# NGWPC/topoflow-glacier

Measured on AMD Instinct MI355X. Metric: cell-updates/sec (nx·ny·steps) on 8192² fp32 grid; % HBM roofline, higher is better.
Workload: dtype f32

## Files before the change

topoflow-glacier_amd/csrc/tfg_fused.hpp:

```cpp
#pragma once

#include <hip/hip_runtime.h>

#include <algorithm>
#include <cmath>
#include <cstddef>
#include <cstdint>

#include "../../include/tfg.h"
#include "tfg_physics.hpp"

namespace tfg_kern {

using tfg::CellDiag;
using tfg::CellOut;
using tfg::CellState;
using tfg::CellStatic;
using tfg::CellStaticF;
using tfg::DevParams;

constexpr int kBlock = 256;
constexpr int kCellsPerThread = 1;
constexpr int kPrefetchFast = 2;
constexpr int kWaves = kBlock / 64;
constexpr int kNumForc = 5;
constexpr int kNumState = 8;
constexpr int kNumHist = 6;
enum { S_HSWE = 0, S_HIWE, S_ECCS, S_ECCI, S_N, S_ALB, S_HSNOW, S_HICE };
enum { F_P = 0, F_T, F_Q, F_PA, F_UZ };
enum { H_HSNOW = 0, H_SM, H_HICE, H_IM, H_MTOT, H_RH };

struct KArgs {
  DevParams p;
  int K;
  int n_catch;
  int64_t n, n_pad;
  const void* io_in;
  double* io_out;
  uint32_t* io_flag;
  uint32_t io_seq;
  int64_t n_step = 0;
  int64_t part_c0 = 0;
};

struct StepAddr {
  int64_t forc, ring, hist, pad_;
};
static_assert(sizeof(StepAddr) == 32, "one aligned scalar load of four dwords reaches forc and ring");

static_assert(offsetof(KArgs, p) == 0, "KArgs::p is read at the start of the kernel-argument segment");
#define TFG_STEP_PARAMS(p)                                                                                  \
  auto p##_ks = (const __attribute__((address_space(4))) DevParams*)__builtin_amdgcn_kernarg_segment_ptr(); \
  asm volatile("" : "+s"(p##_ks));                                                                          \
  const DevParams& p = *(const DevParams*)p##_ks

template <class T, int C> struct alignas(C * sizeof(T)) Pack { T v[C]; };

__device__ __forceinline__ uint32_t lane_off(uint32_t off) {
  asm volatile("" : "+v"(off));
  return off;
}
template <class T, int C>
__device__ __forceinline__ void vload(const T* __restrict__ base, uint32_t i, T (&v)[C]) {
  const uint32_t off = lane_off(i * (uint32_t)sizeof(T));
  const Pack<T, C> x = *reinterpret_cast<const Pack<T, C>*>(reinterpret_cast<const char*>(base) + off);
#pragma unroll
  for (int j = 0; j < C; ++j) v[j] = x.v[j];
}
template <class T, int C>
__device__ __forceinline__ void vstore(T* __restrict__ base, uint32_t i, const T (&v)[C]) {
  const uint32_t off = lane_off(i * (uint32_t)sizeof(T));
  Pack<T, C> x;
#pragma unroll
  for (int j = 0; j < C; ++j) x.v[j] = v[j];
  *reinterpret_cast<Pack<T, C>*>(reinterpret_cast<char*>(base) + off) = x;
}
template <class T>
__device__ __forceinline__ T sload(const T* __restrict__ base, uint32_t off) {
  return *reinterpret_cast<const T*>(reinterpret_cast<const char*>(base) + off);
}
template <class T>
__device__ __forceinline__ void sstore(T* __restrict__ base, uint32_t off, T v) {
  __builtin_nontemporal_store(v, reinterpret_cast<T*>(reinterpret_cast<char*>(base) + off));
}
template <int C> __device__ __forceinline__ void dload(const double* p, uint32_t i, double (&v)[C]) { vload<double, C>(p, i, v); }
template <int C> __device__ __forceinline__ void dstore(double* p, uint32_t i, const double (&v)[C]) { vstore<double, C>(p, i, v); }
template <int C> __device__ __forceinline__ void iload(const int32_t* p, uint32_t i, int32_t (&v)[C]) { vload<int32_t, C>(p, i, v); }
template <int C> __device__ __forceinline__ void istore(int32_t* p, uint32_t i, const int32_t (&v)[C]) { vstore<int32_t, C>(p, i, v); }
template <int C> __device__ __forceinline__ void lload(const int64_t* p, uint32_t i, int64_t (&v)[C]) { vload<int64_t, C>(p, i, v); }
template <int C> __device__ __forceinline__ void lstore(int64_t* p, uint32_t i, const int64_t (&v)[C]) { vstore<int64_t, C>(p, i, v); }

__device__ __forceinline__ void diag_scale(CellDiag& d, const DevParams& p) {
  const double f = p.da_m2 * p.dt, f3600 = p.da_m2 * p.dt * 3600.0;
  d.P *= f;
  d.PR *= f;
  d.PS *= f;
  d.SM *= f3600;
  d.IM *= f3600;
}
__device__ __forceinline__ void diag_zero(CellDiag& d) {
  d.P = d.PR = d.PS = d.SM = d.IM = 0.0;
  d.Pmax = -INFINITY;
}

__device__ __forceinline__ void wave_flush(double* __restrict__ wbins, int cid, const CellDiag& d, bool has) {
  const int lane = threadIdx.x & 63;
  uint64_t pending = __ballot(has);
  while (pending) {
    const int leader = __builtin_ctzll(pending);
    const int c = __shfl(cid, leader);
    const bool mine = has && (cid == c);
    double v0 = mine ? d.P : 0.0, v1 = mine ? d.PR : 0.0, v2 = mine ? d.PS : 0.0;
    double v3 = mine ? d.SM : 0.0, v4 = mine ? d.IM : 0.0, m = mine ? d.Pmax : -INFINITY;
#pragma unroll
    for (int off = 32; off >= 1; off >>= 1) {
      v0 += __shfl_xor(v0, off);
      v1 += __shfl_xor(v1, off);
      v2 += __shfl_xor(v2, off);
      v3 += __shfl_xor(v3, off);
      v4 += __shfl_xor(v4, off);
      m = tfg::npmax(m, __shfl_xor(m, off));
    }
    if (lane == leader) {
      double* b = wbins + 6 * c;
      b[0] += v0; b[1] += v1; b[2] += v2; b[3] += v3; b[4] += v4;
      b[5] = tfg::npmax(b[5], m);
    }
    pending &= ~__ballot(mine);
  }
}

#ifdef TFG_WG_TIMING
static __device__ unsigned long long g_wg_times[TFG_WG_TIMING][3];
#endif
constexpr int kMinWaves = 4;
constexpr int kMinWavesExact = 2;
constexpr int kMinWavesPrec = 4;
template <class R, bool EXACT, bool READ_DEPTHS, bool CATCH, bool QC, int C, bool NS = false, bool PREC = false,
          bool SAT = false>
__global__ __launch_bounds__(kBlock, EXACT ? kMinWavesExact : (PREC ? kMinWavesPrec : kMinWaves)) void k_fused(const KArgs a, const tfg_uniforms* __restrict__ uni,
                                                  const StepAddr* __restrict__ tab,
                                                  const R* __restrict__ forc,
                                                  const R* __restrict__ stat,
                                                  const float* __restrict__ geo,
                                                  const int32_t* __restrict__ catch_id,
                                                  double* __restrict__ st,
                                                  int64_t* __restrict__ tot,
                                                  int32_t* __restrict__ ring,
                                                  R* __restrict__ hist,
                                                  double* __restrict__ slab,
                                                  const R* __restrict__ qcf) {
  extern __shared__ double lds_bins[];
#ifdef TFG_WG_TIMING
  const unsigned long long t_wg0 = wall_clock64();
#endif
  const DevParams& p = a.p;
  const int nb = a.n_catch * 6;
  for (int i = threadIdx.x; i < kWaves * nb; i += kBlock) lds_bins[i] = ((i % 6) == 5) ? -INFINITY : 0.0;
  __syncthreads();
  double* wbins = lds_bins + (threadIdx.x >> 6) * nb;

  const int64_t n_pad = a.n_pad;
  const int64_t ngroups = a.n_step / C;
  const int64_t nchunks = (ngroups + kBlock - 1) / kBlock;
  const int64_t wg = blockIdx.x;
  const int64_t g0 = (wg * nchunks / gridDim.x) * kBlock;
  const int64_t g1 = std::min<int64_t>(((wg + 1) * nchunks / gridDim.x) * kBlock, ngroups);
  const int64_t trips = (g1 - g0 + kBlock - 1) / kBlock;
  const double* geo_d = reinterpret_cast<const double*>(geo + tfg::kGeoF * n_pad) + a.part_c0 / 2;
  float* const alb_f = reinterpret_cast<float*>(st + S_ALB * n_pad) - a.part_c0;

  CellDiag acc;
  diag_zero(acc);

  for (int64_t it = 0; it < trips; ++it) {
    const int64_t g = g0 + it * kBlock + threadIdx.x;
    const bool in = g < g1;
    int32_t cid[C];
    CellDiag cacc[CATCH ? C : 1];
    if constexpr (CATCH) {
#pragma unroll
      for (int j = 0; j < C; ++j) { diag_zero(cacc[j]); cid[j] = 0; }
    }
    if (in) {
      const int64_t c0 = g * C;
      const uint32_t lc = (uint32_t)c0;
      if constexpr (CATCH) iload<C>(catch_id, lc, cid);
      CellStatic SX[EXACT ? C : 1];
      tfg::CellStaticF SF[EXACT ? 1 : C];
      if constexpr (EXACT) {
        const double* gx = reinterpret_cast<const double*>(geo);
        double v[tfg::kStaticPlanes][C];
#pragma unroll
        for (int f = 0; f < tfg::kStaticPlanes; ++f) dload<C>(gx + f * n_pad, lc, v[f]);
#pragma unroll
        for (int j = 0; j < C; ++j) SX[j] = {v[0][j], v[1][j], v[2][j], v[3][j], v[4][j], v[5][j], v[6][j]};
      } else {
        float gv[tfg::kGeoF][C];
#pragma unroll
        for (int f = 0; f < tfg::kGeoF; ++f) vload<float, C>(geo + f * n_pad, lc, gv[f]);
#pragma unroll
        for (int j = 0; j < C; ++j) SF[j] = {gv[0][j], gv[1][j], gv[2][j], gv[3][j], gv[4][j]};
      }
      CellState cs[C];
      {
        double v[C];
        dload<C>(st + S_HSWE * n_pad, lc, v);
#pragma unroll
        for (int j = 0; j < C; ++j) cs[j].h_swe = v[j];
        dload<C>(st + S_HIWE * n_pad, lc, v);
#pragma unroll
        for (int j = 0; j < C; ++j) cs[j].h_iwe = v[j];
        dload<C>(st + S_ECCS * n_pad, lc, v);
#pragma unroll
        for (int j = 0; j < C; ++j) cs[j].Eccs = v[j];
        dload<C>(st + S_ECCI * n_pad, lc, v);
#pragma unroll
        for (int j = 0; j < C; ++j) cs[j].Ecci = v[j];
        dload<C>(st + S_N * n_pad, lc, v);
#pragma unroll
        for (int j = 0; j < C; ++j) cs[j].n = v[j];
        if constexpr (EXACT) {
          dload<C>(st + S_ALB * n_pad, lc, v);
#pragma unroll
          for (int j = 0; j < C; ++j) cs[j].albedo = v[j];
        }
        if constexpr (READ_DEPTHS) {
          dload<C>(st + S_HSNOW * n_pad, lc, v);
#pragma unroll
          for (int j = 0; j < C; ++j) cs[j].h_snow = v[j];
          dload<C>(st + S_HICE * n_pad, lc, v);
#pragma unroll
          for (int j = 0; j < C; ++j) cs[j].h_ice = v[j];
        } else {
#pragma unroll
          for (int j = 0; j < C; ++j) {
            cs[j].h_snow = cs[j].h_swe * p.ws;
            cs[j].h_ice = cs[j].h_iwe * p.wi;
          }
        }
        int64_t t[C];
        lload<C>(tot, lc, t);
#pragma unroll
        for (int j = 0; j < C; ++j) cs[j].tot_q = t[j];
        if constexpr (!EXACT) {
          bool carried = false;
#pragma unroll
          for (int j = 0; j < C; ++j) {
            cs[j].albedo = 0.0;
            carried |= !(cs[j].h_snow > 0.0 || (cs[j].h_snow == 0.0 && (cs[j].h_ice > 0.0 || cs[j].h_ice == 0.0)));
          }
          if (__any(carried)) {
            float fa[C];
            vload<float, C>(alb_f, lc, fa);
#pragma unroll
            for (int j = 0; j < C; ++j) cs[j].albedo = (double)fa[j];
          }
        }
      }
      R qc[C];
      if constexpr (QC) vload<R, C>(qcf, lc, qc);
      else {
#pragma unroll
        for (int j = 0; j < C; ++j) qc[j] = (R)0;
      }
      tfg::DiagF df[EXACT ? 1 : C];
      if constexpr (!EXACT) {
#pragma unroll
        for (int j = 0; j < C; ++j) df[j] = {0.0f, 0.0f, 0.0f, 0.0f, 0.0f, 0.0f};
      }

      struct Frame { R P[C], T[C], Q[C], PA[C], UZ[C]; int32_t q[C]; };
      const char* const fbase = a.io_in ? static_cast<const char*>(a.io_in) : reinterpret_cast<const char*>(forc);
      auto fetch = [&](int k, Frame& f) {
        const StepAddr* ta = tab + (k < a.K ? k : a.K - 1);
        const int64_t fo = ta->forc, ro = ta->ring;
        const R* __restrict__ fr = reinterpret_cast<const R*>(fbase + fo);
        const int32_t* rs = reinterpret_cast<const int32_t*>(reinterpret_cast<const char*>(ring) + ro);
        static_assert(C == 1, "streamed step accesses are per cell");
        static_assert(sizeof(R) == 4 || sizeof(R) == 8, "R is float or double");
        const uint32_t oR = lane_off(lc * (uint32_t)sizeof(R));
        f.P[0] = sload(fr + F_P * n_pad, oR);
        f.T[0] = sload(fr + F_T * n_pad, oR);
        f.Q[0] = sload(fr + F_Q * n_pad, oR);
        f.PA[0] = sload(fr + F_PA * n_pad, oR);
        f.UZ[0] = sload(fr + F_UZ * n_pad, oR);
        f.q[0] = sload(rs, sizeof(R) == 4 ? oR : lane_off(lc * 4u));
      };
      auto advance = [&](int k, const Frame& f) {
        TFG_STEP_PARAMS(p);
        const tfg_uniforms* up = uni + k;
        const tfg_uniforms u = *up;
        int32_t qn[C];
        R o_hs[C], o_sm[C], o_hi[C], o_im[C], o_mt[C], o_rh[C];
#pragma unroll
        for (int j = 0; j < C; ++j) {
          if constexpr (EXACT) {
            CellOut o;
            CellDiag& d = CATCH ? cacc[j] : acc;
            const bool valid = (c0 + j) < a.n;
            const tfg::ParamsAsIs params{p};
            tfg::cell_step_exact<QC>(p, SX[j], u, (double)f.P[j], (double)f.T[j], (double)f.Q[j], (double)f.PA[j],
                                     (double)f.UZ[j], f.q[j], qn[j], cs[j], o, d, valid, (double)qc[j], params);
            o_hs[j] = (R)o.h_snow; o_sm[j] = (R)o.SM; o_hi[j] = (R)o.h_ice;
            o_im[j] = (R)o.IM; o_mt[j] = (R)o.M_total; o_rh[j] = (R)o.RH;
          } else {
            tfg::CellOutF o;
            tfg::cell_step_fast<QC, NS, PREC, SAT>(p, SF[j], up, u, geo_d, n_pad, c0 + j, (float)f.P[j], (float)f.T[j],
                                                   (float)f.Q[j], (float)f.PA[j], (float)f.UZ[j], f.q[j], qn[j], cs[j],
                                                   o, df[j], (float)qc[j]);
            o_hs[j] = (R)o.h_snow; o_sm[j] = (R)o.SM; o_hi[j] = (R)o.h_ice;
            o_im[j] = (R)o.IM; o_mt[j] = (R)o.M_total; o_rh[j] = (R)o.RH;
          }
        }
        const uint32_t oR = lane_off(lc * (uint32_t)sizeof(R));
        const int64_t ro = tab[k].ring, ho = tab[k].hist;
        sstore(reinterpret_cast<int32_t*>(reinterpret_cast<char*>(ring) + ro), sizeof(R) == 4 ? oR : lane_off(lc * 4u), qn[0]);
        R* __restrict__ h = reinterpret_cast<R*>(reinterpret_cast<char*>(hist) + ho);
        sstore(h + H_HSNOW * n_pad, oR, o_hs[0]);
        sstore(h + H_SM * n_pad, oR, o_sm[0]);
        sstore(h + H_HICE * n_pad, oR, o_hi[0]);
        sstore(h + H_IM * n_pad, oR, o_im[0]);
        sstore(h + H_MTOT * n_pad, oR, o_mt[0]);
        sstore(h + H_RH * n_pad, oR, o_rh[0]);
      };
      constexpr int kAhead = (QC || NS || PREC) ? 1 : kPrefetchFast;
      Frame fa, fb;
      fetch(0, fa);
      if constexpr (EXACT) {
        for (int k = 0; k < a.K; ++k) {
          fetch(k + 1, fb);
          advance(k, fa);
          fa = fb;
        }
      } else if constexpr (kAhead == 2) {
        Frame fc;
        fetch(1, fb);
        for (int k = 0; k < a.K; k += 3) {
          fetch(k + 2, fc);
          advance(k, fa);
          fetch(k + 3, fa);
          if (k + 1 < a.K) advance(k + 1, fb);
          fetch(k + 4, fb);
          if (k + 2 < a.K) advance(k + 2, fc);
        }
      } else {
        for (int k = 0; k < a.K; k += 2) {
          fetch(k + 1, fb);
          advance(k, fa);
          fetch(k + 2, fa);
          if (k + 1 < a.K) advance(k + 1, fb);
        }
      }
      if (a.io_in) {
        const int fidx = uni[0].frame, hidx = uni[0].hist;
        R* __restrict__ fr = const_cast<R*>(forc) + (int64_t)fidx * kNumForc * n_pad;
        const uint32_t oR = lane_off(lc * (uint32_t)sizeof(R));
        sstore(fr + F_P * n_pad, oR, fa.P[0]);
        sstore(fr + F_T * n_pad, oR, fa.T[0]);
        sstore(fr + F_Q * n_pad, oR, fa.Q[0]);
        sstore(fr + F_PA * n_pad, oR, fa.PA[0]);
        sstore(fr + F_UZ * n_pad, oR, fa.UZ[0]);
        if (c0 < a.n) {
          const R* hs = hist + (int64_t)hidx * kNumHist * n_pad + c0;
          double* o = a.io_out + c0;
          const int64_t n = a.n;
          o[0 * n] = (double)hs[H_HSNOW * n_pad];
          o[1 * n] = cs[0].h_swe;
          o[2 * n] = (double)hs[H_SM * n_pad];
          o[3 * n] = (double)hs[H_HICE * n_pad];
          o[4 * n] = cs[0].h_iwe;
          o[5 * n] = (double)hs[H_IM * n_pad];
          o[6 * n] = (double)hs[H_MTOT * n_pad];
          o[7 * n] = (double)hs[H_RH * n_pad];
        }
      }
      if constexpr (!EXACT) {
        const double fP = p.da_m2 * p.dt, fSM = p.inv_dt_rhoLf * p.da_m2 * p.dt * 3600.0,
                     fIM = p.da_m2 * p.dt * 3600.0;
#pragma unroll
        for (int j = 0; j < C; ++j) {
          if ((c0 + j) < a.n) {
            CellDiag& d = CATCH ? cacc[j] : acc;
            d.P += (double)df[j].P * fP;
            d.PR += (double)df[j].PR * fP;
            d.PS += (double)df[j].PS * fP;
            d.SM += (double)df[j].Erem_s * fSM;
            d.IM += (double)df[j].IM * fIM;
            d.Pmax = tfg::npmax(d.Pmax, (double)df[j].Pmax);
          }
        }
      }
      {
        double v[C];
#pragma unroll
        for (int j = 0; j < C; ++j) v[j] = cs[j].h_swe;
        dstore<C>(st + S_HSWE * n_pad, lc, v);
#pragma unroll
        for (int j = 0; j < C; ++j) v[j] = cs[j].h_iwe;
        dstore<C>(st + S_HIWE * n_pad, lc, v);
#pragma unroll
        for (int j = 0; j < C; ++j) v[j] = cs[j].Eccs;
        dstore<C>(st + S_ECCS * n_pad, lc, v);
#pragma unroll
        for (int j = 0; j < C; ++j) v[j] = cs[j].Ecci;
        dstore<C>(st + S_ECCI * n_pad, lc, v);
#pragma unroll
        for (int j = 0; j < C; ++j) v[j] = cs[j].n;
        dstore<C>(st + S_N * n_pad, lc, v);
        if constexpr (EXACT) {
#pragma unroll
          for (int j = 0; j < C; ++j) v[j] = cs[j].albedo;
          dstore<C>(st + S_ALB * n_pad, lc, v);
        } else {
          float fa[C];
#pragma unroll
          for (int j = 0; j < C; ++j) fa[j] = (float)cs[j].albedo;
          vstore<float, C>(alb_f, lc, fa);
        }
        int64_t t[C];
#pragma unroll
        for (int j = 0; j < C; ++j) t[j] = cs[j].tot_q;
        lstore<C>(tot, lc, t);
      }
    }
    if constexpr (CATCH) {
#pragma unroll
      for (int j = 0; j < C; ++j) {
        if constexpr (EXACT) diag_scale(cacc[j], p);
        wave_flush(wbins, cid[j], cacc[j], in);
      }
    }
  }
  if constexpr (EXACT && !CATCH) diag_scale(acc, p);
  if constexpr (!CATCH) wave_flush(wbins, 0, acc, true);
  __syncthreads();
  double* bslab = slab + (int64_t)blockIdx.x * nb;
  for (int i = threadIdx.x; i < nb; i += kBlock) {
    double v = lds_bins[i];
    if ((i % 6) == 5) {
      for (int w = 1; w < kWaves; ++w) v = tfg::npmax(v, lds_bins[w * nb + i]);
      bslab[i] = tfg::npmax(bslab[i], v);
    } else {
      for (int w = 1; w < kWaves; ++w) v += lds_bins[w * nb + i];
      bslab[i] += v;
    }
  }
#ifdef TFG_WG_TIMING
  __syncthreads();
  if (threadIdx.x == 0 && blockIdx.x < TFG_WG_TIMING) {
    const unsigned xcc = __builtin_amdgcn_s_getreg((3 << 11) | (0 << 6) | 20);
    g_wg_times[blockIdx.x][0] = t_wg0;
    g_wg_times[blockIdx.x][1] = wall_clock64();
    g_wg_times[blockIdx.x][2] = ((unsigned long long)xcc << 32) | (unsigned)__smid();
  }
#endif
  if (a.io_flag) {
    __threadfence_system();
    __syncthreads();
    if (threadIdx.x == 0)
      __hip_atomic_store(a.io_flag + blockIdx.x, a.io_seq, __ATOMIC_RELEASE, __HIP_MEMORY_SCOPE_SYSTEM);
  }
}

struct FusedBufs {
  const tfg_uniforms* uni;
  const StepAddr* tab;
  const void* forc;
  const void* stat;
  const float* geo;
  const int32_t* catch_id;
  double* st;
  int64_t* tot;
  int32_t* ring;
  void* hist;
  double* slab;
  const void* qc;
};

hipError_t launch_fused_exact(const KArgs& a, const FusedBufs& b, bool read_depths, bool catchments, bool qc_on,
                              int blocks, size_t lds, hipStream_t stream);
template <bool PREC, bool SAT>
hipError_t launch_fused_fast(const KArgs& a, const FusedBufs& b, bool read_depths, bool catchments, bool qc_on,
                             bool nan_safe, int blocks, size_t lds, hipStream_t stream) {
  constexpr int C = kCellsPerThread;
#define TFG_ARGS a, b.uni, b.tab, static_cast<const float*>(b.forc), static_cast<const float*>(b.stat), b.geo, b.catch_id, \
                 b.st, b.tot, b.ring, static_cast<float*>(b.hist), b.slab, static_cast<const float*>(b.qc)
#define TFG_LAUNCH(RD, CT, QC, NS) \
  hipLaunchKernelGGL((k_fused<float, false, RD, CT, QC, C, NS, PREC, SAT>), blocks, kBlock, lds, stream, TFG_ARGS)
#define TFG_LAUNCH_NS(RD, CT, QC) \
  do { if (nan_safe) TFG_LAUNCH(RD, CT, QC, true); else TFG_LAUNCH(RD, CT, QC, false); } while (0)
  if (qc_on) {
    if (read_depths && catchments) TFG_LAUNCH_NS(true, true, true);
    else if (read_depths) TFG_LAUNCH_NS(true, false, true);
    else if (catchments) TFG_LAUNCH_NS(false, true, true);
    else TFG_LAUNCH_NS(false, false, true);
  } else {
    if (read_depths && catchments) TFG_LAUNCH_NS(true, true, false);
    else if (read_depths) TFG_LAUNCH_NS(true, false, false);
    else if (catchments) TFG_LAUNCH_NS(false, true, false);
    else TFG_LAUNCH_NS(false, false, false);
  }
#undef TFG_LAUNCH_NS
#undef TFG_LAUNCH
#undef TFG_ARGS
  return hipGetLastError();
}
extern template hipError_t launch_fused_fast<false, false>(const KArgs&, const FusedBufs&, bool, bool, bool, bool, int,
                                                           size_t, hipStream_t);
extern template hipError_t launch_fused_fast<true, false>(const KArgs&, const FusedBufs&, bool, bool, bool, bool, int,
                                                          size_t, hipStream_t);
extern template hipError_t launch_fused_fast<false, true>(const KArgs&, const FusedBufs&, bool, bool, bool, bool, int,
                                                          size_t, hipStream_t);
extern template hipError_t launch_fused_fast<true, true>(const KArgs&, const FusedBufs&, bool, bool, bool, bool, int,
                                                         size_t, hipStream_t);

}
```

Baseline: 135.2 billion.

## Spill fast-path diag accumulators to LDS and peel the time-step pipeline loops

In the fast, non-catchment variant, the per-thread double diagnostic accumulators now live in shared memory between trips instead of staying in registers, to lower VGPR pressure across the time-step loop. The prefetch/advance loops are peeled so the steady-state body has no tail conditionals, with a separate epilogue for the leftover steps. The catchment-id load is moved to just before it is used, and an empty asm barrier pins some diagnostic values to VGPRs. The costs are extra LDS traffic and 12 KB of shared memory per block, which could reduce occupancy.

```diff
diff --git a/topoflow-glacier_amd/csrc/tfg_fused.hpp b/topoflow-glacier_amd/csrc/tfg_fused.hpp
--- a/topoflow-glacier_amd/csrc/tfg_fused.hpp
+++ b/topoflow-glacier_amd/csrc/tfg_fused.hpp
@@ -172,6 +172,17 @@
 
   CellDiag acc;
   diag_zero(acc);
+  constexpr bool kAccLds = !EXACT && !CATCH;
+  __shared__ double acc_lds[kAccLds ? 6 * kBlock : 1];
+  auto acc_get = [&]() {
+    const double* s = acc_lds + threadIdx.x;
+    return CellDiag{s[0], s[kBlock], s[2 * kBlock], s[3 * kBlock], s[4 * kBlock], s[5 * kBlock]};
+  };
+  auto acc_put = [&](const CellDiag& d) {
+    double* s = acc_lds + threadIdx.x;
+    s[0] = d.P; s[kBlock] = d.PR; s[2 * kBlock] = d.PS; s[3 * kBlock] = d.SM; s[4 * kBlock] = d.IM; s[5 * kBlock] = d.Pmax;
+  };
+  if constexpr (kAccLds) acc_put(acc);
 
   for (int64_t it = 0; it < trips; ++it) {
     const int64_t g = g0 + it * kBlock + threadIdx.x;
@@ -185,7 +196,6 @@
     if (in) {
       const int64_t c0 = g * C;
       const uint32_t lc = (uint32_t)c0;
-      if constexpr (CATCH) iload<C>(catch_id, lc, cid);
       CellStatic SX[EXACT ? C : 1];
       tfg::CellStaticF SF[EXACT ? 1 : C];
       if constexpr (EXACT) {
@@ -311,6 +321,7 @@
                                                    o, df[j], (float)qc[j]);
             o_hs[j] = (R)o.h_snow; o_sm[j] = (R)o.SM; o_hi[j] = (R)o.h_ice;
             o_im[j] = (R)o.IM; o_mt[j] = (R)o.M_total; o_rh[j] = (R)o.RH;
+            asm volatile("" : "+v"(df[j].P), "+v"(df[j].PR), "+v"(df[j].PS), "+v"(df[j].Pmax));
           }
         }
         const uint32_t oR = lane_off(lc * (uint32_t)sizeof(R));
@@ -336,21 +347,49 @@
       } else if constexpr (kAhead == 2) {
         Frame fc;
         fetch(1, fb);
-        for (int k = 0; k < a.K; k += 3) {
-          fetch(k + 2, fc);
+        int k = 0;
+        if (a.K >= 3) {
+          fetch(2, fc);
+          advance(0, fa);
+          fetch(3, fa);
+          advance(1, fb);
+          fetch(4, fb);
+          advance(2, fc);
+          for (k = 3; k + 3 <= a.K; k += 3) {
+            fetch(k + 2, fc);
+            advance(k, fa);
+            fetch(k + 3, fa);
+            advance(k + 1, fb);
+            fetch(k + 4, fb);
+            advance(k + 2, fc);
+          }
+        }
+        if (k < a.K) {
           advance(k, fa);
-          fetch(k + 3, fa);
           if (k + 1 < a.K) advance(k + 1, fb);
-          fetch(k + 4, fb);
-          if (k + 2 < a.K) advance(k + 2, fc);
-        }
-      } else {
+        }
+      } else if constexpr (PREC && CATCH) {
         for (int k = 0; k < a.K; k += 2) {
           fetch(k + 1, fb);
           advance(k, fa);
           fetch(k + 2, fa);
           if (k + 1 < a.K) advance(k + 1, fb);
         }
+      } else {
+        int k = 0;
+        if (a.K >= 2) {
+          fetch(1, fb);
+          advance(0, fa);
+          fetch(2, fa);
+          advance(1, fb);
+          for (k = 2; k + 2 <= a.K; k += 2) {
+            fetch(k + 1, fb);
+            advance(k, fa);
+            fetch(k + 2, fa);
+            advance(k + 1, fb);
+          }
+        }
+        if (k < a.K) advance(k, fa);
       }
       if (a.io_in) {
         const int fidx = uni[0].frame, hidx = uni[0].hist;
@@ -375,19 +414,23 @@
           o[7 * n] = (double)hs[H_RH * n_pad];
         }
       }
+      if constexpr (CATCH) iload<C>(catch_id, lc, cid);
       if constexpr (!EXACT) {
         const double fP = p.da_m2 * p.dt, fSM = p.inv_dt_rhoLf * p.da_m2 * p.dt * 3600.0,
                      fIM = p.da_m2 * p.dt * 3600.0;
 #pragma unroll
         for (int j = 0; j < C; ++j) {
           if ((c0 + j) < a.n) {
-            CellDiag& d = CATCH ? cacc[j] : acc;
+            CellDiag lsum;
+            if constexpr (kAccLds) lsum = acc_get();
+            CellDiag& d = CATCH ? cacc[j] : (kAccLds ? lsum : acc);
             d.P += (double)df[j].P * fP;
             d.PR += (double)df[j].PR * fP;
             d.PS += (double)df[j].PS * fP;
             d.SM += (double)df[j].Erem_s * fSM;
             d.IM += (double)df[j].IM * fIM;
             d.Pmax = tfg::npmax(d.Pmax, (double)df[j].Pmax);
+            if constexpr (kAccLds) acc_put(lsum);
           }
         }
       }
@@ -433,6 +476,7 @@
     }
   }
   if constexpr (EXACT && !CATCH) diag_scale(acc, p);
+  if constexpr (kAccLds) acc = acc_get();
   if constexpr (!CATCH) wave_flush(wbins, 0, acc, true);
   __syncthreads();
   double* bslab = slab + (int64_t)blockIdx.x * nb;
```

New measurement: 137.1 billion, median of 6. No clear change (+1.4%).
